# LinChen-65/pygcn

Measured on AMD Instinct MI355X. Metric: SpMM GEdge/s + fwd+bwd ms/epoch, 10M-node synthetic CSR, feat_dim=256, higher is better.
Workload: dtype f32

## Files before the change

pygcn_amd/csrc/gcn_pack.hip:

```cpp
#include <hip/hip_runtime.h>

#include <cstdint>

#include "gcn_spmm.h"

int gcn_internal_fail(int code, const char *msg);
int gcn_internal_fail_hip(int hip_error, const char *where);

namespace {

constexpr int kWave = 64;
constexpr int kRowsPerBlock = 4;
typedef uint16_t bf16_t;

template <typename T> struct Quad;
template <> struct Quad<float> {
    typedef float4 Raw;
    static __device__ __forceinline__ void load(const float *p, float (&x)[4])
    {
        const float4 v = *(const float4 *)p;
        x[0] = v.x; x[1] = v.y; x[2] = v.z; x[3] = v.w;
    }
    static __device__ __forceinline__ void store(float *p, const float (&x)[4])
    {
        *(float4 *)p = make_float4(x[0], x[1], x[2], x[3]);
    }
};
template <> struct Quad<bf16_t> {
    static __device__ __forceinline__ void load(const bf16_t *p, float (&x)[4])
    {
        const uint2 v = *(const uint2 *)p;
        x[0] = __uint_as_float(v.x << 16); x[1] = __uint_as_float(v.x & 0xffff0000u);
        x[2] = __uint_as_float(v.y << 16); x[3] = __uint_as_float(v.y & 0xffff0000u);
    }
    static __device__ __forceinline__ void store(bf16_t *p, const float (&x)[4])
    {
        uint2 v;
        v.x = (__float_as_uint(x[0]) >> 16) | (__float_as_uint(x[1]) & 0xffff0000u);
        v.y = (__float_as_uint(x[2]) >> 16) | (__float_as_uint(x[3]) & 0xffff0000u);
        *(uint2 *)p = v;
    }
};

__device__ __forceinline__ int below(unsigned long long m)
{
    return (int)__builtin_amdgcn_mbcnt_hi((uint32_t)(m >> 32), __builtin_amdgcn_mbcnt_lo((uint32_t)m, 0u));
}

template <int CTRL> __device__ __forceinline__ uint32_t dpp_u(uint32_t v)
{
    return (uint32_t)__builtin_amdgcn_update_dpp(0, (int)v, CTRL, 0xF, 0xF, true);
}

__device__ __forceinline__ uint32_t or8(uint32_t v)
{
    v |= dpp_u<0xB1>(v);
    v |= dpp_u<0x4E>(v);
    v |= dpp_u<0x141>(v);
    return v;
}

template <typename T>
__global__ __launch_bounds__(kWave *kRowsPerBlock) void pack_count_kernel(
    const T *__restrict__ src, int64_t ld, const int64_t *__restrict__ rows, int64_t m, int F,
    uint32_t *__restrict__ bits, int32_t *__restrict__ counts)
{
    const int lane = threadIdx.x & (kWave - 1);
    const int64_t r = (int64_t)blockIdx.x * kRowsPerBlock + (threadIdx.x >> 6);
    if (r >= m) return;
    const T *row = src + (rows ? rows[r] : r) * ld;
    const int words = F >> 5;
    int cnt = 0;
    for (int f0 = 0; f0 < F; f0 += 4 * kWave) {
        const int f = f0 + 4 * lane;
        uint32_t nib = 0u;
        if (f < F) {
            float x[4];
            Quad<T>::load(row + f, x);
#pragma unroll
            for (int k = 0; k < 4; ++k) nib |= (x[k] != 0.f ? 1u : 0u) << k;
        }
        cnt += __builtin_popcount(nib);
        const uint32_t w = or8(nib << (4 * (lane & 7)));
        if ((lane & 7) == 0 && f < F) bits[r * words + (f >> 5)] = w;
    }
#pragma unroll
    for (int off = 32; off > 0; off >>= 1) cnt += __shfl_xor(cnt, off, kWave);
    if (lane == 0) counts[r] = cnt;
}

template <typename T>
__global__ __launch_bounds__(kWave *kRowsPerBlock) void pack_values_kernel(
    const T *__restrict__ src, int64_t ld, const int64_t *__restrict__ rows, int64_t m, int F,
    const int64_t *__restrict__ offsets, T *__restrict__ vals)
{
    const int lane = threadIdx.x & (kWave - 1);
    const int64_t r = (int64_t)blockIdx.x * kRowsPerBlock + (threadIdx.x >> 6);
    if (r >= m) return;
    const T *row = src + (rows ? rows[r] : r) * ld;
    int64_t base = offsets[r];
    for (int f0 = 0; f0 < F; f0 += 4 * kWave) {
        const int f = f0 + 4 * lane;
        float x[4] = {0.f, 0.f, 0.f, 0.f};
        if (f < F) Quad<T>::load(row + f, x);
        unsigned long long b[4];
        int pos = 0, total = 0;
#pragma unroll
        for (int k = 0; k < 4; ++k) {
            b[k] = __ballot(x[k] != 0.f);
            pos += below(b[k]);
            total += __builtin_popcountll(b[k]);
        }
#pragma unroll
        for (int k = 0; k < 4; ++k) {
            if (x[k] != 0.f) {
                T out;
                if (sizeof(T) == 4) *(float *)&out = x[k];
                else *(bf16_t *)&out = (bf16_t)(__float_as_uint(x[k]) >> 16);
                vals[base + pos] = out;
                ++pos;
            }
        }
        base += total;
    }
}

template <typename T>
__global__ __launch_bounds__(kWave *kRowsPerBlock) void unpack_kernel(
    const uint32_t *__restrict__ bits, const int64_t *__restrict__ offsets, const T *__restrict__ vals,
    int64_t m, int F, T *__restrict__ dst, int64_t ldd)
{
    const int lane = threadIdx.x & (kWave - 1);
    const int64_t r = (int64_t)blockIdx.x * kRowsPerBlock + (threadIdx.x >> 6);
    if (r >= m) return;
    const int words = F >> 5;
    int64_t base = offsets[r];
    for (int f0 = 0; f0 < F; f0 += 4 * kWave) {
        const int f = f0 + 4 * lane;
        uint32_t nib = 0u;
        if (f < F) nib = (bits[r * words + (f >> 5)] >> (4 * (lane & 7))) & 0xFu;
        float x[4];
        int pos = 0, total = 0;
        unsigned long long b[4];
#pragma unroll
        for (int k = 0; k < 4; ++k) {
            b[k] = __ballot(((nib >> k) & 1u) != 0u);
            pos += below(b[k]);
            total += __builtin_popcountll(b[k]);
        }
#pragma unroll
        for (int k = 0; k < 4; ++k) {
            x[k] = 0.f;
            if ((nib >> k) & 1u) {
                const T v = vals[base + pos];
                x[k] = sizeof(T) == 4 ? *(const float *)&v : __uint_as_float((uint32_t)(*(const bf16_t *)&v) << 16);
                ++pos;
            }
        }
        if (f < F) Quad<T>::store(dst + r * ldd + f, x);
        base += total;
    }
}

__global__ __launch_bounds__(256) void bits_count_kernel(const uint32_t *__restrict__ bits, int64_t m, int words,
                                                         int32_t *__restrict__ counts)
{
    const int64_t r = ((int64_t)blockIdx.x * 256 + threadIdx.x) >> 3;
    const int sub = threadIdx.x & 7;
    int c = 0;
    if (r < m)
        for (int w = sub; w < words; w += 8) c += __builtin_popcount(bits[r * words + w]);
    c += __shfl_xor(c, 1, kWave);
    c += __shfl_xor(c, 2, kWave);
    c += __shfl_xor(c, 4, kWave);
    if (r < m && sub == 0) counts[r] = c;
}

constexpr int kPack512Cap = GCN_PACK512_CAPACITY;

__device__ __forceinline__ uint32_t or16(uint32_t v)
{
    v = or8(v);
    v |= dpp_u<0x140>(v);
    return v;
}

__global__ __launch_bounds__(kWave *kRowsPerBlock) void pack512_kernel(const float *__restrict__ src, int64_t ld,
                                                                       int64_t m, uint32_t *__restrict__ slots)
{
    const int lane = threadIdx.x & (kWave - 1);
    const int64_t r = (int64_t)blockIdx.x * kRowsPerBlock + (threadIdx.x >> 6);
    if (r >= m) return;
    const int q = lane >> 4, i = lane & 15;
    const uint4 v = *(const uint4 *)(src + r * ld + 16 * i + 4 * q);
    const uint32_t x[4] = {v.x, v.y, v.z, v.w};
    uint32_t nib = 0u;
#pragma unroll
    for (int j = 0; j < 4; ++j) nib |= (x[j] != 0u ? 1u : 0u) << j;
    const uint32_t lo = or16(i < 8 ? nib << (4 * i) : 0u), hi = or16(i >= 8 ? nib << (4 * (i - 8)) : 0u);
    const unsigned long long mask = ((unsigned long long)hi << 32) | lo;
    int rank = __builtin_popcountll(mask & ((1ull << (4 * i)) - 1ull));
    uint32_t *sub = slots + r * 128 + 32 * q;
    if (i == 0) {
        sub[0] = lo;
        sub[1] = hi;
        sub[2] = (uint32_t)__builtin_popcountll(mask);
    }
#pragma unroll
    for (int j = 0; j < 4; ++j) {
        if ((nib >> j) & 1u) {
            if (rank < kPack512Cap) sub[3 + rank] = x[j];
            ++rank;
        }
    }
}

int check(const char *who, int dtype, int64_t m, int64_t F, int64_t ld)
{
    if (dtype != GCN_DTYPE_F32 && dtype != GCN_DTYPE_BF16) return gcn_internal_fail(GCN_E_BADARG, who);
    if (m < 0 || F <= 0 || F % 32 != 0 || F > INT32_MAX || ld < F || ld % 4 != 0)
        return gcn_internal_fail(GCN_E_BADARG, who);
    return 0;
}

}

extern "C" {

int gcn_rows_pack_count(int dtype, const void *src, int64_t ld, const int64_t *rows, int64_t m, int64_t F,
                        uint32_t *bits, int32_t *counts, void *stream)
{
    if (int rc = check("gcn_rows_pack_count: bad dtype / sizes (F a multiple of 32, ld a multiple of 4)", dtype, m, F, ld))
        return rc;
    if (m == 0) return 0;
    if (src == nullptr || bits == nullptr || counts == nullptr)
        return gcn_internal_fail(GCN_E_BADARG, "gcn_rows_pack_count: NULL pointer");
    if (((uintptr_t)src) % 16 != 0) return gcn_internal_fail(GCN_E_ALIGN, "gcn_rows_pack_count: 16-byte alignment required");
    const dim3 grid((unsigned)((m + kRowsPerBlock - 1) / kRowsPerBlock)), block(kWave * kRowsPerBlock);
    hipStream_t s = (hipStream_t)stream;
    if (dtype == GCN_DTYPE_F32)
        hipLaunchKernelGGL(pack_count_kernel<float>, grid, block, 0, s, (const float *)src, ld, rows, m, (int)F, bits, counts);
    else
        hipLaunchKernelGGL(pack_count_kernel<bf16_t>, grid, block, 0, s, (const bf16_t *)src, ld, rows, m, (int)F, bits, counts);
    hipError_t e = hipGetLastError();
    return e == hipSuccess ? 0 : gcn_internal_fail_hip((int)e, "gcn_rows_pack_count launch");
}

int gcn_rows_pack_values(int dtype, const void *src, int64_t ld, const int64_t *rows, int64_t m, int64_t F,
                         const int64_t *offsets, void *vals, void *stream)
{
    if (int rc = check("gcn_rows_pack_values: bad dtype / sizes (F a multiple of 32, ld a multiple of 4)", dtype, m, F, ld))
        return rc;
    if (m == 0) return 0;
    if (src == nullptr || offsets == nullptr || vals == nullptr)
        return gcn_internal_fail(GCN_E_BADARG, "gcn_rows_pack_values: NULL pointer");
    if (((uintptr_t)src) % 16 != 0) return gcn_internal_fail(GCN_E_ALIGN, "gcn_rows_pack_values: 16-byte alignment required");
    const dim3 grid((unsigned)((m + kRowsPerBlock - 1) / kRowsPerBlock)), block(kWave * kRowsPerBlock);
    hipStream_t s = (hipStream_t)stream;
    if (dtype == GCN_DTYPE_F32)
        hipLaunchKernelGGL(pack_values_kernel<float>, grid, block, 0, s, (const float *)src, ld, rows, m, (int)F, offsets, (float *)vals);
    else
        hipLaunchKernelGGL(pack_values_kernel<bf16_t>, grid, block, 0, s, (const bf16_t *)src, ld, rows, m, (int)F, offsets, (bf16_t *)vals);
    hipError_t e = hipGetLastError();
    return e == hipSuccess ? 0 : gcn_internal_fail_hip((int)e, "gcn_rows_pack_values launch");
}

int gcn_rows_unpack(int dtype, const uint32_t *bits, const int64_t *offsets, const void *vals, int64_t m,
                    int64_t F, void *dst, int64_t ldd, void *stream)
{
    if (int rc = check("gcn_rows_unpack: bad dtype / sizes (F a multiple of 32, ldd a multiple of 4)", dtype, m, F, ldd))
        return rc;
    if (m == 0) return 0;
    if (bits == nullptr || offsets == nullptr || dst == nullptr)
        return gcn_internal_fail(GCN_E_BADARG, "gcn_rows_unpack: NULL pointer");
    if (((uintptr_t)dst) % 16 != 0) return gcn_internal_fail(GCN_E_ALIGN, "gcn_rows_unpack: 16-byte alignment required");
    const dim3 grid((unsigned)((m + kRowsPerBlock - 1) / kRowsPerBlock)), block(kWave * kRowsPerBlock);
    hipStream_t s = (hipStream_t)stream;
    if (dtype == GCN_DTYPE_F32)
        hipLaunchKernelGGL(unpack_kernel<float>, grid, block, 0, s, bits, offsets, (const float *)vals, m, (int)F, (float *)dst, ldd);
    else
        hipLaunchKernelGGL(unpack_kernel<bf16_t>, grid, block, 0, s, bits, offsets, (const bf16_t *)vals, m, (int)F, (bf16_t *)dst, ldd);
    hipError_t e = hipGetLastError();
    return e == hipSuccess ? 0 : gcn_internal_fail_hip((int)e, "gcn_rows_unpack launch");
}

int gcn_rows_pack512(const float *src, int64_t ld, int64_t m, uint32_t *slots, void *stream)
{
    if (m < 0 || ld < 256 || ld % 4 != 0) return gcn_internal_fail(GCN_E_BADARG, "gcn_rows_pack512: bad sizes (256 columns, ld a multiple of 4)");
    if (m == 0) return 0;
    if (src == nullptr || slots == nullptr) return gcn_internal_fail(GCN_E_BADARG, "gcn_rows_pack512: NULL pointer");
    if ((((uintptr_t)src) | ((uintptr_t)slots)) % 16 != 0)
        return gcn_internal_fail(GCN_E_ALIGN, "gcn_rows_pack512: 16-byte alignment required");
    if ((m + kRowsPerBlock - 1) / kRowsPerBlock > INT32_MAX) return gcn_internal_fail(GCN_E_BADARG, "gcn_rows_pack512: too many rows");
    const dim3 grid((unsigned)((m + kRowsPerBlock - 1) / kRowsPerBlock)), block(kWave * kRowsPerBlock);
    hipLaunchKernelGGL(pack512_kernel, grid, block, 0, (hipStream_t)stream, src, ld, m, slots);
    hipError_t e = hipGetLastError();
    return e == hipSuccess ? 0 : gcn_internal_fail_hip((int)e, "gcn_rows_pack512 launch");
}

int gcn_bits_row_counts(const uint32_t *bits, int64_t m, int64_t words, int32_t *counts, void *stream)
{
    if (m < 0 || words <= 0 || words > (1 << 20))
        return gcn_internal_fail(GCN_E_BADARG, "gcn_bits_row_counts: bad sizes");
    if (m == 0) return 0;
    if (bits == nullptr || counts == nullptr) return gcn_internal_fail(GCN_E_BADARG, "gcn_bits_row_counts: NULL pointer");
    const dim3 grid((unsigned)((m * 8 + 255) / 256)), block(256);
    hipLaunchKernelGGL(bits_count_kernel, grid, block, 0, (hipStream_t)stream, bits, m, (int)words, counts);
    hipError_t e = hipGetLastError();
    return e == hipSuccess ? 0 : gcn_internal_fail_hip((int)e, "gcn_bits_row_counts launch");
}

}
```

pygcn_amd/csrc/gcn_spmm.hip:

```cpp
#include <hip/hip_runtime.h>

#include <algorithm>
#include <climits>
#include <cstdint>
#include <cstdio>
#include <cstring>
#include <type_traits>

#include "gcn_spmm.h"

static inline uint32_t gcn_dropout_threshold16(float p)
{
    if (!(p > 0.f)) return 0u;
    const double t = (double)p * 65536.0 + 0.5;
    return (uint32_t)std::min(65535.0, std::max(1.0, (double)(int64_t)t));
}
static inline float gcn_dropout_scale16(uint32_t thresh)
{
    return thresh == 0u ? 1.f : 65536.f / (float)(65536u - thresh);
}

namespace {

constexpr int kWave = 64;
// ... 173 lines not shown
            const int ws = idx >> 5;
            const uint32_t w = (ws & 2) ? ((ws & 1) ? r[3] : r[2]) : ((ws & 1) ? r[1] : r[0]);
            const uint32_t nib = w >> (idx & 31);
#pragma unroll
            for (int j = 0; j < (VEC == 1 ? 1 : 4); ++j)
                o[4 * q + j] = ((nib >> j) & 1u) ? o[4 * q + j] * p.drop_scale : 0.f;
        }
        return;
    }
    if (VEC == 1) {
        const uint32_t blk = ((uint32_t)(f >> 4) << 1) | ((uint32_t)(f >> 2) & 1u);
        const int fld = (((f >> 3) & 1) << 2) | (f & 3);
        philox4x32_10((uint32_t)row, (uint32_t)(row >> 32), blk, 0u, k0, k1, r);
        const uint32_t w = (fld & 4) ? ((fld & 2) ? r[3] : r[2]) : ((fld & 2) ? r[1] : r[0]);
        const uint32_t bits = (fld & 1) ? (w >> 16) : (w & 0xFFFFu);
        o[0] = (bits >= p.drop_thresh) ? o[0] * p.drop_scale : 0.f;
    } else {
#pragma unroll
        for (int q = 0; q < VEC / 4; ++q) {
            const int fq = f + 4 * q;
            const uint32_t blk = ((uint32_t)(fq >> 4) << 1) | ((uint32_t)(fq >> 2) & 1u);
            philox4x32_10((uint32_t)row, (uint32_t)(row >> 32), blk, 0u, k0, k1, r);
            const bool hi = ((fq >> 3) & 1) != 0;
            const uint32_t w0 = hi ? r[2] : r[0], w1 = hi ? r[3] : r[1];
            o[4 * q + 0] = ((w0 & 0xFFFFu) >= p.drop_thresh) ? o[4 * q + 0] * p.drop_scale : 0.f;
            o[4 * q + 1] = ((w0 >> 16) >= p.drop_thresh) ? o[4 * q + 1] * p.drop_scale : 0.f;
            o[4 * q + 2] = ((w1 & 0xFFFFu) >= p.drop_thresh) ? o[4 * q + 2] * p.drop_scale : 0.f;
            o[4 * q + 3] = ((w1 >> 16) >= p.drop_thresh) ? o[4 * q + 3] * p.drop_scale : 0.f;
        }
    }
}

template <int CTRL>
__device__ __forceinline__ float dpp_move(float v)
{
    return __int_as_float(__builtin_amdgcn_update_dpp(0, __float_as_int(v), CTRL, 0xF, 0xF, true));
}

template <int LPR>
__device__ __forceinline__ float group_max(float m)
{
    if (LPR >= 2) m = fmaxf(m, dpp_move<0xB1>(m));
    if (LPR >= 4) m = fmaxf(m, dpp_move<0x4E>(m));
    if (LPR >= 8) m = fmaxf(m, dpp_move<0x141>(m));
    if (LPR >= 16) m = fmaxf(m, dpp_move<0x140>(m));
#pragma unroll
    for (int off = 16; off < LPR; off <<= 1) m = fmaxf(m, __shfl_xor(m, off, kWave));
    return m;
}

template <int LPR>
__device__ __forceinline__ float group_sum(float s)
{
    if (LPR >= 2) s += dpp_move<0xB1>(s);
    if (LPR >= 4) s += dpp_move<0x4E>(s);
    if (LPR >= 8) s += dpp_move<0x141>(s);
    if (LPR >= 16) s += dpp_move<0x140>(s);
#pragma unroll
    for (int off = 16; off < LPR; off <<= 1) s += __shfl_xor(s, off, kWave);
    return s;
}

template <typename T, int VEC, int LPR, int XEPI, bool ALLOW_SKIP = true>
__device__ __forceinline__ uint32_t store_out(const KParams &p, int64_t row, int f, bool act,
                                              const float (&acc)[VEC], const float (&bias)[VEC])
{
    float o[VEC];
#pragma unroll
    for (int i = 0; i < VEC; ++i) {
        o[i] = acc[i] + bias[i];
        if (p.relu) o[i] = fmaxf(o[i], 0.f);
    }
    if (p.drop_thresh != 0u) apply_dropout<VEC>(p, row, f, o);
    if (XEPI >= 1 && p.log_softmax) {
        const bool valid = f < p.F;
        float m = -INFINITY;
#pragma unroll
        for (int i = 0; i < VEC; ++i) m = valid ? fmaxf(m, o[i]) : m;
        m = group_max<LPR>(m);
        float se = 0.f;
#pragma unroll
        for (int i = 0; i < VEC; ++i) se += valid ? __expf(o[i] - m) : 0.f;
        se = group_sum<LPR>(se);
        const float lse = m + __logf(se);
#pragma unroll
        for (int i = 0; i < VEC; ++i) o[i] -= lse;
    }
    bool do_store = act;
    if (XEPI >= 2 && p.cflag != nullptr) {
        bool nz = false;
#pragma unroll
        for (int i = 0; i < VEC; ++i) nz |= (o[i] != 0.f);
        if (ALLOW_SKIP && p.cskip) {
            const unsigned long long b = __ballot(act && nz);
            const int ln = (int)(threadIdx.x & (kWave - 1));
            const unsigned long long gm =
                LPR >= kWave ? ~0ull : (((1ull << LPR) - 1ull) << (ln & ~(LPR - 1)));
            do_store = act && (b & gm) != 0ull;
        }
        if (act && nz) p.cflag[row] = 1;
    }
    if (do_store) {
        T *dst = (T *)p.C + row * p.ldc + f;
        *(typename Elem<T, VEC>::Raw *)dst = Elem<T, VEC>::pack(o);
    }
    uint32_t amax = 0u;
    if (XEPI >= 2 && p.cabsmax != nullptr && do_store) {
        float st[VEC];
        Elem<T, VEC>::unpack(Elem<T, VEC>::pack(o), st);
#pragma unroll
        for (int i = 0; i < VEC; ++i)
            if (f + i < p.F) amax = max(amax, __float_as_uint(st[i]) & 0x7fffffffu);
    }
    return amax;
}

template <int XEPI>
__device__ __forceinline__ void publish_absmax(const KParams &p, uint32_t amax)
{
    if (XEPI >= 2 && p.cabsmax != nullptr) {
#pragma unroll
        for (int off = 32; off > 0; off >>= 1) amax = max(amax, (uint32_t)__shfl_xor((int)amax, off, kWave));
        if ((threadIdx.x & (kWave - 1)) == 0 && amax != 0u &&
            amax > __atomic_load_n(p.cabsmax, __ATOMIC_RELAXED))
            atomicMax(p.cabsmax, amax);
    }
}

__device__ __forceinline__ u32x4 row_load16(uint64_t base, uint32_t nbytes, uint32_t voff)
{
    const uint32_t lo = __builtin_amdgcn_readfirstlane((uint32_t)base);
    const uint32_t hi = __builtin_amdgcn_readfirstlane((uint32_t)(base >> 32));
    void *pb = (void *)(((uint64_t)hi << 32) | lo);
    __amdgpu_buffer_rsrc_t rsrc = __builtin_amdgcn_make_buffer_rsrc(pb, 0, nbytes, 0x00020000);
    return __builtin_amdgcn_raw_buffer_load_b128(rsrc, voff, 0, 0);
}

template <typename T, int VEC, int D, bool ROWS, bool FLAGS, int XEPI>
__device__ __forceinline__ void wide_stream(const KParams &p, const int32_t *__restrict__ colp,
                                            const float *__restrict__ valp, int ne, int lane,
                                            unsigned ld_off_bytes, float (&acc)[VEC],
                                            int rel_end, int nr, int64_t row0, int f, bool act,
                                            const float (&bias)[VEC], uint32_t &amax)
{
    typedef typename Elem<T, VEC>::Raw Raw;
    static_assert(sizeof(Raw) == 16, "wide kernel moves 16 bytes per lane");
    const uint32_t ldb_bytes = (uint32_t)(p.ldb * (int64_t)sizeof(T));
    const uint32_t ldb2_bytes = (uint32_t)(p.ldb2 * (int64_t)sizeof(T));
    const uint32_t row_bytes = (uint32_t)p.F * (uint32_t)sizeof(T);
    auto row_base = [&](int c) -> uint64_t {
        return c < p.b_split ? (uint64_t)p.B + (uint64_t)(uint32_t)c * ldb_bytes
                             : (uint64_t)p.B2 + (uint64_t)(uint32_t)(c - p.b_split) * ldb2_bytes;
    };
    int r = 0;
    int rend = ROWS ? readlane_i(rel_end, 0) : INT_MAX;
    const bool flags = FLAGS && use_row_flags(p, 3, 4);
    const bool sel = FLAGS && ROWS && p.csel != nullptr;
    const int want = (sel && lane < nr) ? (int)row_bit(p.csel, (int)row0 + lane) : 1;
    auto emit = [&](int rr) {
        if (!sel || readlane_i(want, rr))
            amax = max(amax, store_out<T, VEC, kWave, XEPI>(p, row0 + rr, f, act, acc, bias));
    };
    auto consume = [&](int e, const u32x4 &raw, float a) {
        if (ROWS) {
            while (e >= rend) {
                emit(r);
#pragma unroll
                for (int i = 0; i < VEC; ++i) acc[i] = 0.f;
                ++r;
                rend = readlane_i(rel_end, r);
            }
        }
        float x[VEC];
        Elem<T, VEC>::unpack(__builtin_bit_cast(Raw, raw), x);
#pragma unroll
        for (int i = 0; i < VEC; ++i) acc[i] = fmaf(a, x[i], acc[i]);
    };

    for (int t = 0; t < ne; t += kWave) {
        const int cnt = min(kWave, ne - t);
        int cv = 0;
        float vv = 0.f;
        if (lane < cnt) {
            cv = colp[t + lane];
            vv = valp[t + lane];
        }
        if (FLAGS && (flags || sel)) {
            int fv = (lane < cnt) ? 1 : 0;
            if (flags) fv = fv && row_bit(p.bflag, cv);
            if (sel) {
                const int i = t + lane;
                int lo = 0, hi = nr - 1;
#pragma unroll
                for (int s = 0; s < 6; ++s) {
                    const int mid = (lo + hi) >> 1;
                    const int v = __shfl(rel_end, mid, kWave);
                    if (v > i) hi = mid; else lo = min(mid + 1, nr - 1);
                }
                const int w = __shfl(want, lo, kWave);
                fv &= w;
            }
            unsigned long long m = __ballot(fv != 0);
            while (m) {
                int kk[D];
                u32x4 x[D];
#pragma unroll
                for (int j = 0; j < D; ++j) {
                    kk[j] = m ? (int)__builtin_ctzll(m) : -1;
                    m &= m - 1;
                    const int c = readlane_i(cv, kk[j] < 0 ? 0 : kk[j]);
                    x[j] = row_load16(row_base(c), kk[j] >= 0 ? row_bytes : 0u, ld_off_bytes);
                }
#pragma unroll
                for (int j = 0; j < D; ++j)
                    if (kk[j] >= 0) consume(t + kk[j], x[j], readlane_f(vv, kk[j]));
            }
            continue;
        }
        for (int k = 0; k < cnt; k += D) {
            u32x4 x[D];
#pragma unroll
            for (int j = 0; j < D; ++j) {
                const bool ok = k + j < cnt;
                const int c = readlane_i(cv, k + j);
                x[j] = row_load16(row_base(c), ok ? row_bytes : 0u, ld_off_bytes);
            }
#pragma unroll
            for (int j = 0; j < D; ++j)
                consume(min(t + k + j, ne - 1), x[j], readlane_f(vv, k + j));
        }
    }
    if (ROWS) {
        while (r < nr) {
            emit(r);
#pragma unroll
            for (int i = 0; i < VEC; ++i) acc[i] = 0.f;
            ++r;
        }
    }
}

template <typename T, int VEC, typename IdxT, int D, bool FLAGS, int XEPI>
__global__ __launch_bounds__(kWave *kWavesPerBlock) void spmm_wide_kernel(KParams p)
{
    const int lane = threadIdx.x & (kWave - 1);
    const int item =
        blockIdx.x * kWavesPerBlock + __builtin_amdgcn_readfirstlane((int)(threadIdx.x >> 6));
    if (item >= p.n_total) return;
    const int f = blockIdx.y * (kWave * VEC) + lane * VEC;
    const bool act = f < p.F;
    const unsigned ld_off_bytes = (unsigned)f * (unsigned)sizeof(T);
    const IdxT *__restrict__ rp = (const IdxT *)p.rowptr;

    float acc[VEC], bias[VEC];
#pragma unroll
    for (int i = 0; i < VEC; ++i) {
        acc[i] = 0.f;
        bias[i] = 0.f;
    }

    if (item < p.n_chunks) {
        const int row = p.chunk_row[item];
        if (FLAGS && p.csel != nullptr && !row_bit(p.csel, row)) return;
        const int64_t e0 = p.chunk_e0[item];
        const int64_t e1 = min(e0 + (int64_t)p.long_thresh, (int64_t)rp[row + 1]);
        uint32_t unused = 0u;
        wide_stream<T, VEC, D, false, FLAGS, XEPI>(p, p.col + e0, p.val + e0, (int)(e1 - e0), lane,
                                      ld_off_bytes, acc, 0, 0, 0, f, act, bias, unused);
        if (act) {
            float *dst = p.partial + (int64_t)item * p.F + f;
#pragma unroll
            for (int i = 0; i < VEC; ++i) dst[i] = acc[i];
        }
        return;
    }

    const int it = item - p.n_chunks;
    const int ra = p.items[2 * it], rb = p.items[2 * it + 1];
    const int nr = rb - ra;
    const int64_t ea = (int64_t)rp[ra];
    const int rel_end = (lane < nr) ? (int)((int64_t)rp[ra + 1 + lane] - ea) : 0;
    const int ne = readlane_i(rel_end, nr - 1);
    if (p.bias != nullptr && act) {
#pragma unroll
        for (int i = 0; i < VEC; ++i) bias[i] = p.bias[f + i];
    }
    uint32_t amax = 0u;
    wide_stream<T, VEC, D, true, FLAGS, XEPI>(p, p.col + ea, p.val + ea, ne, lane, ld_off_bytes, acc, rel_end,
                                 nr, (int64_t)ra, f, act, bias, amax);
    publish_absmax<XEPI>(p, amax);
}

typedef uint32_t u32x2 __attribute__((ext_vector_type(2)));

__device__ __forceinline__ u32x2 slot_load8(uint64_t base, uint32_t nbytes, uint32_t voff)
{
    const uint32_t lo = __builtin_amdgcn_readfirstlane((uint32_t)base);
    const uint32_t hi = __builtin_amdgcn_readfirstlane((uint32_t)(base >> 32));
    void *pb = (void *)(((uint64_t)hi << 32) | lo);
    __amdgpu_buffer_rsrc_t rsrc = __builtin_amdgcn_make_buffer_rsrc(pb, 0, nbytes, 0x00020000);
    return __builtin_amdgcn_raw_buffer_load_b64(rsrc, voff, 0, 0);
}

template <int N> __device__ __forceinline__ uint32_t row_bcast(uint32_t v)
{
    return (uint32_t)__builtin_amdgcn_mov_dpp((int)v, 0x150 + N, 0xF, 0xF, true);
}

constexpr int kPackSlotBytes = 512;
constexpr uint32_t kPackCap = GCN_PACK512_CAPACITY;

template <int D, bool ROWS>
__device__ __forceinline__ void packed_stream(const KParams &p, const int32_t *__restrict__ colp,
                                              const float *__restrict__ valp, int ne, int lane, float (&acc)[4],
                                              int rel_end, int nr, int64_t row0, int f, const float (&bias)[4])
{
    const int i = lane & 15;
    const uint32_t ldb_bytes = (uint32_t)(p.ldb * 4);
    const uint32_t voff = (uint32_t)lane * 8u;
    const unsigned long long below = (1ull << (4 * i)) - 1ull;
    const int row_lane0 = (lane & 48) << 2;
    int r = 0;
    int rend = ROWS ? readlane_i(rel_end, 0) : INT_MAX;
    auto consume = [&](int e, const u32x2 &raw, float a, int c) {
        if (ROWS) {
            while (e >= rend) {
                store_out<float, 4, kWave, 0>(p, row0 + r, f, true, acc, bias);
#pragma unroll
                for (int k = 0; k < 4; ++k) acc[k] = 0.f;
                ++r;
                rend = readlane_i(rel_end, r);
            }
        }
        const uint32_t mlo = row_bcast<0>(raw.x), mhi = row_bcast<0>(raw.y), cnt = row_bcast<1>(raw.x);
        float x[4];
        if (__ballot(cnt > kPackCap) != 0ull) {
            const u32x4 d = row_load16((uint64_t)p.B + (uint64_t)(uint32_t)c * ldb_bytes, 1024u, (uint32_t)f * 4u);
            Elem<float, 4>::unpack(__builtin_bit_cast(f32x4, d), x);
        } else {
            const unsigned long long m = ((unsigned long long)mhi << 32) | mlo;
            const uint32_t nib = (uint32_t)(m >> (4 * i)) & 0xFu;
            const int w0 = 3 + __builtin_popcountll(m & below);
            const int w2 = w0 << 1;
            const int a0 = row_lane0 | (w2 & 60), a1 = row_lane0 | ((w2 + 4) & 60), a2 = row_lane0 | ((w2 + 8) & 60);
            const int s0 = __builtin_amdgcn_ds_bpermute(a0, (int)raw.x), s1 = __builtin_amdgcn_ds_bpermute(a0, (int)raw.y);
            const int s2 = __builtin_amdgcn_ds_bpermute(a1, (int)raw.x), s3 = __builtin_amdgcn_ds_bpermute(a1, (int)raw.y);
            const int s4 = __builtin_amdgcn_ds_bpermute(a2, (int)raw.x);
            const bool odd = (w0 & 1) != 0;
            float q0 = __int_as_float(odd ? s1 : s0), q1 = __int_as_float(odd ? s2 : s1),
                  q2 = __int_as_float(odd ? s3 : s2), q3 = __int_as_float(odd ? s4 : s3);
            const bool b0 = (nib & 1u) != 0u, b1 = (nib & 2u) != 0u, b2 = (nib & 4u) != 0u, b3 = (nib & 8u) != 0u;
            x[0] = b0 ? q0 : 0.f;
            q0 = b0 ? q1 : q0; q1 = b0 ? q2 : q1; q2 = b0 ? q3 : q2;
            x[1] = b1 ? q0 : 0.f;
            q0 = b1 ? q1 : q0; q1 = b1 ? q2 : q1;
            x[2] = b2 ? q0 : 0.f;
            q0 = b2 ? q1 : q0;
            x[3] = b3 ? q0 : 0.f;
        }
#pragma unroll
        for (int k = 0; k < 4; ++k) acc[k] = fmaf(a, x[k], acc[k]);
    };

    for (int t = 0; t < ne; t += kWave) {
        const int cnt = min(kWave, ne - t);
        int cv = 0;
        float vv = 0.f;
        if (lane < cnt) {
            cv = colp[t + lane];
            vv = valp[t + lane];
        }
        for (int k = 0; k < cnt; k += D) {
            u32x2 x[D];
            int cc[D];
#pragma unroll
            for (int j = 0; j < D; ++j) {
                const bool ok = k + j < cnt;
                cc[j] = readlane_i(cv, k + j);
                x[j] = slot_load8((uint64_t)p.packed + (uint64_t)(uint32_t)cc[j] * (uint64_t)kPackSlotBytes,
                                  ok ? (uint32_t)kPackSlotBytes : 0u, voff);
            }
#pragma unroll
            for (int j = 0; j < D; ++j)
                consume(min(t + k + j, ne - 1), x[j], readlane_f(vv, k + j), cc[j]);
        }
    }
    if (ROWS) {
        while (r < nr) {
            store_out<float, 4, kWave, 0>(p, row0 + r, f, true, acc, bias);
#pragma unroll
            for (int k = 0; k < 4; ++k) acc[k] = 0.f;
            ++r;
        }
    }
}

template <typename IdxT, int D>
__global__ __launch_bounds__(kWave *kWavesPerBlock) void spmm_wide_packed_kernel(KParams p)
{
    const int lane = threadIdx.x & (kWave - 1);
    const int item =
        blockIdx.x * kWavesPerBlock + __builtin_amdgcn_readfirstlane((int)(threadIdx.x >> 6));
    if (item >= p.n_total) return;
    const int f = 16 * (lane & 15) + 4 * (lane >> 4);
    const IdxT *__restrict__ rp = (const IdxT *)p.rowptr;
    float acc[4] = {0.f, 0.f, 0.f, 0.f}, bias[4] = {0.f, 0.f, 0.f, 0.f};

    if (item < p.n_chunks) {
        const int row = p.chunk_row[item];
        const int64_t e0 = p.chunk_e0[item];
        const int64_t e1 = min(e0 + (int64_t)p.long_thresh, (int64_t)rp[row + 1]);
        packed_stream<D, false>(p, p.col + e0, p.val + e0, (int)(e1 - e0), lane, acc, 0, 0, 0, f, bias);
        float *dst = p.partial + (int64_t)item * p.F + f;
#pragma unroll
        for (int k = 0; k < 4; ++k) dst[k] = acc[k];
        return;
    }
    const int it = item - p.n_chunks;
    const int ra = p.items[2 * it], rb = p.items[2 * it + 1];
    const int nr = rb - ra;
    const int64_t ea = (int64_t)rp[ra];
    const int rel_end = (lane < nr) ? (int)((int64_t)rp[ra + 1 + lane] - ea) : 0;
    const int ne = readlane_i(rel_end, nr - 1);
    if (p.bias != nullptr) {
#pragma unroll
        for (int k = 0; k < 4; ++k) bias[k] = p.bias[f + k];
    }
    packed_stream<D, true>(p, p.col + ea, p.val + ea, ne, lane, acc, rel_end, nr, (int64_t)ra, f, bias);
}

template <typename T>
__device__ __forceinline__ const char *narrow_row_ptr(const KParams &p, int c)
{
    return c < p.b_split ? (const char *)p.B + (int64_t)c * (p.ldb * (int64_t)sizeof(T))
                         : (const char *)p.B2 + (int64_t)(c - p.b_split) * (p.ldb2 * (int64_t)sizeof(T));
}

template <typename T, int VEC, int LPR, int U>
__device__ __forceinline__ void narrow_row(const KParams &p, const int32_t *__restrict__ col,
                                           const float *__restrict__ val, int64_t e0, int64_t e1,
                                           int g, unsigned ld_off, float (&acc)[VEC],
                                           bool flags = false)
{
    typedef typename Elem<T, VEC>::Raw Raw;
    constexpr int G = kWave / LPR;
    if (flags) {
        const int lane = (int)(threadIdx.x & (kWave - 1));
        for (int64_t t = e0; t < e1; t += kWave) {
            const int cnt = (int)min((int64_t)kWave, e1 - t);
            int c = 0;
            float a = 0.f;
            bool keep = false;
            if (lane < cnt) {
                c = col[t + lane];
                a = val[t + lane];
                keep = row_bit(p.bflag, c);
            }
            const unsigned long long m = __ballot(keep);
            const int nv = __builtin_popcountll(m);
            if (nv == 0) continue;
            const int below = (int)__builtin_amdgcn_mbcnt_hi((unsigned)(m >> 32),
                                                           __builtin_amdgcn_mbcnt_lo((unsigned)m, 0u));
            const int dest = keep ? below : nv + (lane - below);
            const int cc = __builtin_amdgcn_ds_permute(dest << 2, c);
            const float aa = __int_as_float(__builtin_amdgcn_ds_permute(dest << 2, __float_as_int(a)));
            for (int k = 0; k < nv; k += G * U) {
                Raw x[U];
                float w[U];
#pragma unroll
                for (int u = 0; u < U; ++u) {
                    const int idx = k + u * G + g;
                    const bool ok = idx < nv;
                    const int ck = __shfl(cc, idx & (kWave - 1), kWave);
                    const float ak = __shfl(aa, idx & (kWave - 1), kWave);
                    w[u] = ok ? ak : 0.f;
                    Raw z = {};
                    x[u] = z;
                    if (ok) x[u] = *(const Raw *)(narrow_row_ptr<T>(p, ck) + ld_off);
                }
#pragma unroll
                for (int u = 0; u < U; ++u) {
                    float xf[VEC];
                    Elem<T, VEC>::unpack(x[u], xf);
#pragma unroll
                    for (int i = 0; i < VEC; ++i) acc[i] = fmaf(w[u], xf[i], acc[i]);
                }
            }
        }
    } else
    for (int64_t e = e0; e < e1; e += (int64_t)G * U) {
        int c[U];
        float a[U];
        Raw x[U];
#pragma unroll
        for (int u = 0; u < U; ++u) {
            const int64_t ee = e + (int64_t)u * G + g;
            const bool ok = ee < e1;
            c[u] = ok ? col[ee] : 0;
            a[u] = ok ? val[ee] : 0.f;
        }
#pragma unroll
        for (int u = 0; u < U; ++u) {
            x[u] = *(const Raw *)(narrow_row_ptr<T>(p, c[u]) + ld_off);
        }
#pragma unroll
        for (int u = 0; u < U; ++u) {
            const int64_t ee = e + (int64_t)u * G + g;
            if (ee < e1) {
                float xf[VEC];
                Elem<T, VEC>::unpack(x[u], xf);
#pragma unroll
                for (int i = 0; i < VEC; ++i) acc[i] = fmaf(a[u], xf[i], acc[i]);
            }
        }
    }
    if (G > 1) {
#pragma unroll
        for (int off = LPR; off < kWave; off <<= 1) {
#pragma unroll
            for (int i = 0; i < VEC; ++i) acc[i] += __shfl_xor(acc[i], off, kWave);
        }
    }
}

template <typename T, int VEC, int LPR, typename IdxT, int XEPI>
__global__ __launch_bounds__(kWave *kWavesPerBlock) void spmm_narrow_kernel(KParams p)
{
    constexpr int U = 4;
    const int lane = threadIdx.x & (kWave - 1);
    const int item =
        blockIdx.x * kWavesPerBlock + __builtin_amdgcn_readfirstlane((int)(threadIdx.x >> 6));
    if (item >= p.n_total) return;
    const int g = lane / LPR, l = lane % LPR;
    const int f = blockIdx.y * (LPR * VEC) + l * VEC;
    const bool act = f < p.F;
    const unsigned ld_off = act ? (unsigned)f * (unsigned)sizeof(T) : 0u;
    const IdxT *__restrict__ rp = (const IdxT *)p.rowptr;
    const bool flags = use_row_flags(p, 1, 8);

    float acc[VEC], bias[VEC];
#pragma unroll
    for (int i = 0; i < VEC; ++i) {
        acc[i] = 0.f;
        bias[i] = 0.f;
    }

    const bool sel = p.csel != nullptr;
    uint32_t amax = 0u;
    if (item < p.n_chunks) {
        const int row = p.chunk_row[item];
        if (sel && !row_bit(p.csel, row)) return;
        const int64_t e0 = p.chunk_e0[item];
        const int64_t e1 = min(e0 + (int64_t)p.long_thresh, (int64_t)rp[row + 1]);
        narrow_row<T, VEC, LPR, U>(p, p.col, p.val, e0, e1, g, ld_off, acc, flags);
        if (act && g == 0) {
            float *dst = p.partial + (int64_t)item * p.F + f;
#pragma unroll
            for (int i = 0; i < VEC; ++i) dst[i] = acc[i];
        }
        return;
    }

    const int it = item - p.n_chunks;
    const int ra = p.items[2 * it], rb = p.items[2 * it + 1];
    const int nr = rb - ra;
    if (p.bias != nullptr && act) {
#pragma unroll
        for (int i = 0; i < VEC; ++i) bias[i] = p.bias[f + i];
    }
    constexpr int G = kWave / LPR;
    const int64_t ea = (int64_t)rp[ra];
    const int rel_end = (lane < nr) ? (int)((int64_t)rp[ra + 1 + lane] - ea) : 0;
    const int ne = readlane_i(rel_end, nr - 1);

    if (G == 1 || nr == 1 || ne > kWave) {
        int64_t e0 = ea;
        for (int r = ra; r < rb; ++r) {
            const int64_t e1 = (int64_t)rp[r + 1];
            if (sel && !row_bit(p.csel, r)) {
                e0 = e1;
                continue;
            }
#pragma unroll
            for (int i = 0; i < VEC; ++i) acc[i] = 0.f;
            narrow_row<T, VEC, LPR, U>(p, p.col, p.val, e0, e1, g, ld_off, acc, flags);
            amax = max(amax, store_out<T, VEC, LPR, XEPI>(p, (int64_t)r, f, act && g == 0, acc, bias));
            e0 = e1;
        }
        publish_absmax<XEPI>(p, amax);
        return;
    }

    typedef typename Elem<T, VEC>::Raw Raw;
    constexpr int RU = 2;
    constexpr int UU = 2;
    constexpr int kShort = 8;
    const int64_t ldb_bytes = p.ldb * (int64_t)sizeof(T);
    int cv = 0;
    float vv = 0.f;
    if (lane < ne) {
        cv = p.col[ea + lane];
        vv = p.val[ea + lane];
        if (flags && !row_bit(p.bflag, cv)) vv = 0.f, cv = -1;
    }
    const int up = __shfl_up(rel_end, 1, kWave);
    const int rel_start = (lane == 0) ? 0 : up;
    const int wantn = (sel && lane < nr) ? (int)row_bit(p.csel, ra + lane) : 1;
    unsigned long long medium = __ballot(lane < nr && rel_end - rel_start > kShort && wantn != 0);

    for (int q0 = 0; q0 < nr; q0 += G * RU) {
        int e0[RU], e1[RU], row[RU];
        float a2[RU][VEC];
#pragma unroll
        for (int ru = 0; ru < RU; ++ru) {
            const int r = q0 + ru * G + g;
            const int s0 = __shfl(rel_start, r & (kWave - 1), kWave);
            const int s1 = __shfl(rel_end, r & (kWave - 1), kWave);
            const int wr = __shfl(wantn, r & (kWave - 1), kWave);
            const bool mine = r < nr && s1 - s0 <= kShort && wr != 0;
            row[ru] = mine ? r : -1;
            e0[ru] = s0;
            e1[ru] = mine ? s1 : s0;
#pragma unroll
            for (int i = 0; i < VEC; ++i) a2[ru][i] = 0.f;
        }
        for (int j = 0; j < kShort; j += UU) {
            bool more = false;
#pragma unroll
            for (int ru = 0; ru < RU; ++ru) more |= (e0[ru] + j < e1[ru]);
            if (!__any(more)) break;
            Raw x[RU][UU];
            float av[RU][UU];
#pragma unroll
            for (int ru = 0; ru < RU; ++ru) {
#pragma unroll
                for (int u = 0; u < UU; ++u) {
                    const int idx = e0[ru] + j + u;
                    const int c = __shfl(cv, idx & (kWave - 1), kWave);
                    const bool ok = idx < e1[ru] && c >= 0;
                    const float a = __shfl(vv, idx & (kWave - 1), kWave);
                    av[ru][u] = ok ? a : 0.f;
                    Raw z = {};
                    x[ru][u] = z;
                    if (ok)
                        x[ru][u] = *(const Raw *)(narrow_row_ptr<T>(p, c) + ld_off);
                }
            }
#pragma unroll
            for (int ru = 0; ru < RU; ++ru) {
#pragma unroll
                for (int u = 0; u < UU; ++u) {
                    float xf[VEC];
                    Elem<T, VEC>::unpack(x[ru][u], xf);
#pragma unroll
                    for (int i = 0; i < VEC; ++i) a2[ru][i] = fmaf(av[ru][u], xf[i], a2[ru][i]);
                }
            }
        }
#pragma unroll
        for (int ru = 0; ru < RU; ++ru) {
            if (row[ru] >= 0)
                amax = max(amax, store_out<T, VEC, LPR, XEPI>(p, (int64_t)(ra + row[ru]), f, act, a2[ru], bias));
        }
    }

    while (medium) {
        const int rr = __builtin_ctzll(medium);
        medium &= medium - 1;
        const int s0 = readlane_i(rel_start, rr), s1 = readlane_i(rel_end, rr);
#pragma unroll
        for (int i = 0; i < VEC; ++i) acc[i] = 0.f;
        narrow_row<T, VEC, LPR, U>(p, p.col, p.val, ea + s0, ea + s1, g, ld_off, acc, flags);
        amax = max(amax, store_out<T, VEC, LPR, XEPI>(p, (int64_t)(ra + rr), f, act && g == 0, acc, bias));
    }
    publish_absmax<XEPI>(p, amax);
}

__device__ __forceinline__ float long_row_sum(const float *__restrict__ partial, int F, int f, int c0, int c1)
{
    float s[16];
#pragma unroll
    for (int k = 0; k < 16; ++k) s[k] = 0.f;
    int c = c0;
    for (; c + 16 <= c1; c += 16) {
#pragma unroll
        for (int k = 0; k < 16; ++k) s[k] += partial[(int64_t)(c + k) * F + f];
    }
#pragma unroll
    for (int k = 0; k < 15; ++k)
        if (c + k < c1) s[k] += partial[(int64_t)(c + k) * F + f];
    return (((s[0] + s[1]) + (s[2] + s[3])) + ((s[4] + s[5]) + (s[6] + s[7]))) +
           (((s[8] + s[9]) + (s[10] + s[11])) + ((s[12] + s[13]) + (s[14] + s[15])));
}

template <typename T>
__global__ __launch_bounds__(256) void spmm_long_reduce_kernel(KParams p)
{
    const int lane = threadIdx.x & (kWave - 1);
    const int j = blockIdx.x * 4 + __builtin_amdgcn_readfirstlane((int)(threadIdx.x >> 6));
    if (j >= p.n_long) return;
    const int64_t row = p.long_row[j];
    if (p.csel != nullptr && !row_bit(p.csel, (int)row)) return;
    const int c0 = p.long_chunk0[j], c1 = p.long_chunk0[j + 1];
    uint32_t amax = 0u;
    if (p.log_softmax) {
        auto col = [&](int k) { return lane + kWave * k; };
        float z[8], m = -INFINITY;
#pragma unroll
        for (int k = 0; k < 8; ++k) {
            const int f = col(k);
            z[k] = -INFINITY;
            if (f < p.F) z[k] = long_row_sum(p.partial, p.F, f, c0, c1) + (p.bias ? p.bias[f] : 0.f);
            m = fmaxf(m, z[k]);
        }
#pragma unroll
        for (int off = 1; off < kWave; off <<= 1) m = fmaxf(m, __shfl_xor(m, off, kWave));
        float se = 0.f;
#pragma unroll
        for (int k = 0; k < 8; ++k) se += (col(k) < p.F) ? expf(z[k] - m) : 0.f;
#pragma unroll
        for (int off = 1; off < kWave; off <<= 1) se += __shfl_xor(se, off, kWave);
        const float lse = m + logf(se);
#pragma unroll
        for (int k = 0; k < 8; ++k) {
            const int f = col(k);
            if (f < p.F) {
                const float o[1] = {z[k] - lse};
                ((T *)p.C)[row * p.ldc + f] = Elem<T, 1>::pack(o);
                if (p.cflag != nullptr && o[0] != 0.f) p.cflag[row] = 1;
                float st[1];
                Elem<T, 1>::unpack(Elem<T, 1>::pack(o), st);
// ... 858 lines not shown
```

Baseline: 7.930.

## Stage packed slots through LDS instead of DPP/bpermute decoding in SpMM

The packed-slot SpMM consumer now writes each fetched 512-byte slot image into per-wave shared memory and decodes masks and compacted values with plain LDS reads, replacing the row-broadcast DPP and multiple ds_bpermute calls. The overflow check is made once per batch with a ballot, and the kernel gets a waves-per-EU occupancy hint. The pack kernel also handles two rows per wave and assembles the slot in LDS before writing it out as coalesced 8-byte stores. The goal is to cut cross-lane shuffle overhead and scattered global stores, at the cost of extra LDS traffic, wave barriers and LDS capacity per block.

```diff
diff --git a/pygcn_amd/csrc/gcn_pack.hip b/pygcn_amd/csrc/gcn_pack.hip
--- a/pygcn_amd/csrc/gcn_pack.hip
+++ b/pygcn_amd/csrc/gcn_pack.hip
@@ -185,32 +185,55 @@
     return v;
 }
 
+#ifndef GCN_PACK512_ROWS_PER_WAVE
+#define GCN_PACK512_ROWS_PER_WAVE 2
+#endif
+constexpr int kPack512RowsPerWave = GCN_PACK512_ROWS_PER_WAVE;
+constexpr int kPack512RowsPerBlock = kRowsPerBlock * kPack512RowsPerWave;
+
 __global__ __launch_bounds__(kWave *kRowsPerBlock) void pack512_kernel(const float *__restrict__ src, int64_t ld,
                                                                        int64_t m, uint32_t *__restrict__ slots)
 {
+    constexpr int R = kPack512RowsPerWave;
+    __shared__ __attribute__((aligned(16))) uint32_t image_all[kRowsPerBlock * R * 128];
     const int lane = threadIdx.x & (kWave - 1);
-    const int64_t r = (int64_t)blockIdx.x * kRowsPerBlock + (threadIdx.x >> 6);
-    if (r >= m) return;
+    const int wave = __builtin_amdgcn_readfirstlane((int)(threadIdx.x >> 6));
+    const int64_t r0 = ((int64_t)blockIdx.x * kRowsPerBlock + wave) * R;
+    if (r0 >= m) return;
+    const int nr = (int)(m - r0 < R ? m - r0 : R);
     const int q = lane >> 4, i = lane & 15;
-    const uint4 v = *(const uint4 *)(src + r * ld + 16 * i + 4 * q);
-    const uint32_t x[4] = {v.x, v.y, v.z, v.w};
-    uint32_t nib = 0u;
-#pragma unroll
-    for (int j = 0; j < 4; ++j) nib |= (x[j] != 0u ? 1u : 0u) << j;
-    const uint32_t lo = or16(i < 8 ? nib << (4 * i) : 0u), hi = or16(i >= 8 ? nib << (4 * (i - 8)) : 0u);
-    const unsigned long long mask = ((unsigned long long)hi << 32) | lo;
-    int rank = __builtin_popcountll(mask & ((1ull << (4 * i)) - 1ull));
-    uint32_t *sub = slots + r * 128 + 32 * q;
-    if (i == 0) {
-        sub[0] = lo;
-        sub[1] = hi;
-        sub[2] = (uint32_t)__builtin_popcountll(mask);
-    }
-#pragma unroll
-    for (int j = 0; j < 4; ++j) {
-        if ((nib >> j) & 1u) {
-            if (rank < kPack512Cap) sub[3 + rank] = x[j];
-            ++rank;
+    uint32_t *image = image_all + wave * (R * 128);
+    uint4 v[R];
+#pragma unroll
+    for (int k = 0; k < R; ++k)
+        v[k] = *(const uint4 *)(src + (r0 + (k < nr ? k : nr - 1)) * ld + 16 * i + 4 * q);
+#pragma unroll
+    for (int k = 0; k < R; ++k) {
+        const uint32_t x[4] = {v[k].x, v[k].y, v[k].z, v[k].w};
+        uint32_t nib = 0u;
+#pragma unroll
+        for (int j = 0; j < 4; ++j) nib |= (x[j] != 0u ? 1u : 0u) << j;
+        const uint32_t lo = or16(i < 8 ? nib << (4 * i) : 0u), hi = or16(i >= 8 ? nib << (4 * (i - 8)) : 0u);
+        const unsigned long long mask = ((unsigned long long)hi << 32) | lo;
+        int rank = __builtin_popcountll(mask & ((1ull << (4 * i)) - 1ull));
+        uint32_t *sub = image + k * 128 + 32 * q;
+        if (i < 3) sub[i] = i == 0 ? lo : i == 1 ? hi : (uint32_t)__builtin_popcountll(mask);
+#pragma unroll
+        for (int j = 0; j < 4; ++j) {
+            if ((nib >> j) & 1u) {
+                if (rank < kPack512Cap) sub[3 + rank] = x[j];
+                ++rank;
+            }
+        }
+    }
+    __builtin_amdgcn_fence(__ATOMIC_RELEASE, "wavefront");
+    __builtin_amdgcn_wave_barrier();
+    __builtin_amdgcn_fence(__ATOMIC_ACQUIRE, "wavefront");
+#pragma unroll
+    for (int k = 0; k < R; ++k) {
+        if (k < nr) {
+            const uint2 w = *(const uint2 *)(image + k * 128 + 2 * lane);
+            *(uint2 *)(slots + (r0 + k) * 128 + 2 * lane) = w;
         }
     }
 }
@@ -291,8 +314,9 @@
     if (src == nullptr || slots == nullptr) return gcn_internal_fail(GCN_E_BADARG, "gcn_rows_pack512: NULL pointer");
     if ((((uintptr_t)src) | ((uintptr_t)slots)) % 16 != 0)
         return gcn_internal_fail(GCN_E_ALIGN, "gcn_rows_pack512: 16-byte alignment required");
-    if ((m + kRowsPerBlock - 1) / kRowsPerBlock > INT32_MAX) return gcn_internal_fail(GCN_E_BADARG, "gcn_rows_pack512: too many rows");
-    const dim3 grid((unsigned)((m + kRowsPerBlock - 1) / kRowsPerBlock)), block(kWave * kRowsPerBlock);
+    const int64_t blocks = (m + kPack512RowsPerBlock - 1) / kPack512RowsPerBlock;
+    if (blocks > INT32_MAX) return gcn_internal_fail(GCN_E_BADARG, "gcn_rows_pack512: too many rows");
+    const dim3 grid((unsigned)blocks), block(kWave * kRowsPerBlock);
     hipLaunchKernelGGL(pack512_kernel, grid, block, 0, (hipStream_t)stream, src, ld, m, slots);
     hipError_t e = hipGetLastError();
     return e == hipSuccess ? 0 : gcn_internal_fail_hip((int)e, "gcn_rows_pack512 launch");
diff --git a/pygcn_amd/csrc/gcn_spmm.hip b/pygcn_amd/csrc/gcn_spmm.hip
--- a/pygcn_amd/csrc/gcn_spmm.hip
+++ b/pygcn_amd/csrc/gcn_spmm.hip
@@ -499,61 +499,69 @@
     return __builtin_amdgcn_raw_buffer_load_b64(rsrc, voff, 0, 0);
 }
 
-template <int N> __device__ __forceinline__ uint32_t row_bcast(uint32_t v)
-{
-    return (uint32_t)__builtin_amdgcn_mov_dpp((int)v, 0x150 + N, 0xF, 0xF, true);
-}
-
 constexpr int kPackSlotBytes = 512;
 constexpr uint32_t kPackCap = GCN_PACK512_CAPACITY;
+constexpr int kStageWords = 168;
+constexpr int kStageTailWords = 32;
+template <int D> constexpr int stage_block_words() { return kWavesPerBlock * D * kStageWords + kStageTailWords; }
+
+__device__ __forceinline__ void wave_sync()
+{
+    __builtin_amdgcn_fence(__ATOMIC_RELEASE, "wavefront");
+    __builtin_amdgcn_wave_barrier();
+    __builtin_amdgcn_fence(__ATOMIC_ACQUIRE, "wavefront");
+}
 
 template <int D, bool ROWS>
-__device__ __forceinline__ void packed_stream(const KParams &p, const int32_t *__restrict__ colp,
+__device__ __forceinline__ void packed_stream(const KParams &p, uint32_t *stage, const int32_t *__restrict__ colp,
                                               const float *__restrict__ valp, int ne, int lane, float (&acc)[4],
                                               int rel_end, int nr, int64_t row0, int f, const float (&bias)[4])
 {
-    const int i = lane & 15;
+    const int q = lane >> 4, i = lane & 15;
     const uint32_t ldb_bytes = (uint32_t)(p.ldb * 4);
     const uint32_t voff = (uint32_t)lane * 8u;
-    const unsigned long long below = (1ull << (4 * i)) - 1ull;
-    const int row_lane0 = (lane & 48) << 2;
+    uint32_t *const sub = stage + 42 * q + 6 * (q & 1);
+    uint32_t *const mine = sub + 2 * i;
+    const bool upper = i >= 8;
+    const uint32_t sh = 4u * (uint32_t)(i & 7);
+    const uint32_t below_lo = upper ? ~0u : (1u << sh) - 1u, below_hi = upper ? (1u << sh) - 1u : 0u;
+    const bool cnt_lane = i == 1;
     int r = 0;
     int rend = ROWS ? readlane_i(rel_end, 0) : INT_MAX;
-    auto consume = [&](int e, const u32x2 &raw, float a, int c) {
+    auto emit = [&](int rr) {
+        store_out<float, 4, kWave, 0>(p, row0 + rr, f, true, acc, bias);
+#pragma unroll
+        for (int k = 0; k < 4; ++k) acc[k] = 0.f;
+    };
+    auto expand = [](uint32_t nibs, const uint32_t (&v)[4], float (&x)[4]) {
+        uint32_t b[4];
+#pragma unroll
+        for (int k = 0; k < 4; ++k) b[k] = (uint32_t)__builtin_amdgcn_sbfe((int)nibs, (uint32_t)k, 1u);
+        auto sel = [](uint32_t m, uint32_t yes, uint32_t no) {
+            uint32_t d;
+            asm("v_bfi_b32 %0, %1, %2, %3" : "=v"(d) : "v"(m), "v"(yes), "v"(no));
+            return d;
+        };
+        uint32_t q0 = v[0], q1 = v[1], q2 = v[2];
+        x[0] = __uint_as_float(q0 & b[0]);
+        q0 = sel(b[0], q1, q0); q1 = sel(b[0], q2, q1); q2 = sel(b[0], v[3], q2);
+        x[1] = __uint_as_float(q0 & b[1]);
+        q0 = sel(b[1], q1, q0); q1 = sel(b[1], q2, q1);
+        x[2] = __uint_as_float(q0 & b[2]);
+        q0 = sel(b[2], q1, q0);
+        x[3] = __uint_as_float(q0 & b[3]);
+    };
+    auto consume = [&](int e, float (&x)[4], bool over, float a, int c) {
         if (ROWS) {
             while (e >= rend) {
-                store_out<float, 4, kWave, 0>(p, row0 + r, f, true, acc, bias);
-#pragma unroll
-                for (int k = 0; k < 4; ++k) acc[k] = 0.f;
+                emit(r);
                 ++r;
                 rend = readlane_i(rel_end, r);
             }
         }
-        const uint32_t mlo = row_bcast<0>(raw.x), mhi = row_bcast<0>(raw.y), cnt = row_bcast<1>(raw.x);
-        float x[4];
-        if (__ballot(cnt > kPackCap) != 0ull) {
+        if (over) {
             const u32x4 d = row_load16((uint64_t)p.B + (uint64_t)(uint32_t)c * ldb_bytes, 1024u, (uint32_t)f * 4u);
             Elem<float, 4>::unpack(__builtin_bit_cast(f32x4, d), x);
-        } else {
-            const unsigned long long m = ((unsigned long long)mhi << 32) | mlo;
-            const uint32_t nib = (uint32_t)(m >> (4 * i)) & 0xFu;
-            const int w0 = 3 + __builtin_popcountll(m & below);
-            const int w2 = w0 << 1;
-            const int a0 = row_lane0 | (w2 & 60), a1 = row_lane0 | ((w2 + 4) & 60), a2 = row_lane0 | ((w2 + 8) & 60);
-            const int s0 = __builtin_amdgcn_ds_bpermute(a0, (int)raw.x), s1 = __builtin_amdgcn_ds_bpermute(a0, (int)raw.y);
-            const int s2 = __builtin_amdgcn_ds_bpermute(a1, (int)raw.x), s3 = __builtin_amdgcn_ds_bpermute(a1, (int)raw.y);
-            const int s4 = __builtin_amdgcn_ds_bpermute(a2, (int)raw.x);
-            const bool odd = (w0 & 1) != 0;
-            float q0 = __int_as_float(odd ? s1 : s0), q1 = __int_as_float(odd ? s2 : s1),
-                  q2 = __int_as_float(odd ? s3 : s2), q3 = __int_as_float(odd ? s4 : s3);
-            const bool b0 = (nib & 1u) != 0u, b1 = (nib & 2u) != 0u, b2 = (nib & 4u) != 0u, b3 = (nib & 8u) != 0u;
-            x[0] = b0 ? q0 : 0.f;
-            q0 = b0 ? q1 : q0; q1 = b0 ? q2 : q1; q2 = b0 ? q3 : q2;
-            x[1] = b1 ? q0 : 0.f;
-            q0 = b1 ? q1 : q0; q1 = b1 ? q2 : q1;
-            x[2] = b2 ? q0 : 0.f;
-            q0 = b2 ? q1 : q0;
-            x[3] = b3 ? q0 : 0.f;
         }
 #pragma unroll
         for (int k = 0; k < 4; ++k) acc[k] = fmaf(a, x[k], acc[k]);
@@ -577,23 +585,65 @@
                 x[j] = slot_load8((uint64_t)p.packed + (uint64_t)(uint32_t)cc[j] * (uint64_t)kPackSlotBytes,
                                   ok ? (uint32_t)kPackSlotBytes : 0u, voff);
             }
-#pragma unroll
-            for (int j = 0; j < D; ++j)
-                consume(min(t + k + j, ne - 1), x[j], readlane_f(vv, k + j), cc[j]);
+            wave_sync();
+            uint32_t top = 0u;
+#pragma unroll
+            for (int j = 0; j < D; ++j) {
+                *(u32x2 *)(mine + j * kStageWords) = x[j];
+                top = max(top, x[j].x);
+            }
+            const bool any_over = __ballot(cnt_lane && top > kPackCap) != 0ull;
+            wave_sync();
+            constexpr int kMaskGroup = 4, kValueGroup = 2;
+            static_assert(D % kMaskGroup == 0 && kMaskGroup % kValueGroup == 0, "groups");
+#pragma unroll
+            for (int g0 = 0; g0 < D; g0 += kMaskGroup) {
+                uint32_t nibs[kMaskGroup];
+                const uint32_t *first[kMaskGroup];
+                u32x2 h[kMaskGroup];
+                wave_sync();
+#pragma unroll
+                for (int j = 0; j < kMaskGroup; ++j) h[j] = *(const u32x2 *)(sub + (g0 + j) * kStageWords);
+#pragma unroll
+                for (int j = 0; j < kMaskGroup; ++j) {
+                    nibs[j] = (upper ? h[j].y : h[j].x) >> sh;
+                    int w0 = __builtin_popcount(h[j].x & below_lo) + __builtin_popcount(h[j].y & below_hi);
+                    asm("" : "+v"(w0));
+                    first[j] = sub + (g0 + j) * kStageWords + 3 + w0;
+                }
+#pragma unroll
+                for (int g = 0; g < kMaskGroup; g += kValueGroup) {
+                    uint32_t v[kValueGroup][4];
+                    float xs[kValueGroup][4];
+                    wave_sync();
+#pragma unroll
+                    for (int j = 0; j < kValueGroup; ++j)
+#pragma unroll
+                        for (int w = 0; w < 4; ++w) v[j][w] = first[g + j][w];
+#pragma unroll
+                    for (int j = 0; j < kValueGroup; ++j) expand(nibs[g + j], v[j], xs[j]);
+#pragma unroll
+                    for (int j = 0; j < kValueGroup; ++j) {
+                        const int e = g0 + g + j;
+                        consume(min(t + k + e, ne - 1), xs[j],
+                                any_over && __ballot(sub[e * kStageWords + 2] > kPackCap) != 0ull,
+                                readlane_f(vv, k + e), cc[e]);
+                    }
+                }
+            }
         }
     }
     if (ROWS) {
         while (r < nr) {
-            store_out<float, 4, kWave, 0>(p, row0 + r, f, true, acc, bias);
-#pragma unroll
-            for (int k = 0; k < 4; ++k) acc[k] = 0.f;
+            emit(r);
             ++r;
         }
     }
 }
 
 template <typename IdxT, int D>
-__global__ __launch_bounds__(kWave *kWavesPerBlock) void spmm_wide_packed_kernel(KParams p)
+__global__ __launch_bounds__(kWave *kWavesPerBlock) __attribute__((amdgpu_waves_per_eu(7, 8)))
+void spmm_wide_packed_kernel(KParams p)
 {
     const int lane = threadIdx.x & (kWave - 1);
     const int item =
@@ -602,12 +652,14 @@
     const int f = 16 * (lane & 15) + 4 * (lane >> 4);
     const IdxT *__restrict__ rp = (const IdxT *)p.rowptr;
     float acc[4] = {0.f, 0.f, 0.f, 0.f}, bias[4] = {0.f, 0.f, 0.f, 0.f};
+    __shared__ __attribute__((aligned(16))) uint32_t stage_all[stage_block_words<D>()];
+    uint32_t *stage = stage_all + __builtin_amdgcn_readfirstlane((int)(threadIdx.x >> 6)) * (D * kStageWords);
 
     if (item < p.n_chunks) {
         const int row = p.chunk_row[item];
         const int64_t e0 = p.chunk_e0[item];
         const int64_t e1 = min(e0 + (int64_t)p.long_thresh, (int64_t)rp[row + 1]);
-        packed_stream<D, false>(p, p.col + e0, p.val + e0, (int)(e1 - e0), lane, acc, 0, 0, 0, f, bias);
+        packed_stream<D, false>(p, stage, p.col + e0, p.val + e0, (int)(e1 - e0), lane, acc, 0, 0, 0, f, bias);
         float *dst = p.partial + (int64_t)item * p.F + f;
 #pragma unroll
         for (int k = 0; k < 4; ++k) dst[k] = acc[k];
@@ -623,7 +675,7 @@
 #pragma unroll
         for (int k = 0; k < 4; ++k) bias[k] = p.bias[f + k];
     }
-    packed_stream<D, true>(p, p.col + ea, p.val + ea, ne, lane, acc, rel_end, nr, (int64_t)ra, f, bias);
+    packed_stream<D, true>(p, stage, p.col + ea, p.val + ea, ne, lane, acc, rel_end, nr, (int64_t)ra, f, bias);
 }
 
 template <typename T>
```

New measurement: 8.348 (median of 6 runs). 5.3% higher.
